# zzhuolun/conditioned-nerf-gan

Measured on AMD Instinct MI355X. Metric: rays/sec at 128x128x64spp ShapeNetCar, higher is better.
Workload: dtype f32; 1 GPU; ImplicitGenerator3d.forward SHORTSIREN_FG hidden 256, 128x128 rays x 64 coarse + 64 fine samples, feature volume 32x64^3, batch 8/GPU, hierarchical, white_back, relu, nerf_noise 0.0; img_size=128, num_steps=64, images_per_gpu=8, parallelism=image-batch data parallel x1, no data-path collective

## Files before the change

### conditioned-nerf-gan_amd/_lib.py

```python
import ctypes as C
import os

HERE = os.path.dirname(os.path.abspath(__file__))
LIB_PATH = os.path.join(HERE, "libcnerf_hip.so")

MAX_LAYERS = 16
MAX_LEVELS = 4
ABI_VERSION = 10
F_HIERARCHICAL, F_WHITE_BACK, F_LAST_BACK, F_SOFTPLUS, F_SIGMOID_RGB, F_INPUT_XYZ = 1, 2, 4, 8, 16, 32
F_NO_VOLUME = 128
PREC_FP32, PREC_FP16, PREC_FP16X3 = 0, 1, 2
PREC_CODE = {"fp32": PREC_FP32, "fp16": PREC_FP16, "fp16x3": PREC_FP16X3}
LAYER_FILM, LAYER_SINE, LAYER_RES, LAYER_PFILM = 0, 1, 2, 3
LAYER_CODE = {"film": LAYER_FILM, "sine": LAYER_SINE, "res": LAYER_RES, "pfilm": LAYER_PFILM}


class Cfg(C.Structure):
    _fields_ = [("B", C.c_int32), ("R", C.c_int32), ("S", C.c_int32), ("V", C.c_int32), ("C", C.c_int32),
                ("H", C.c_int32), ("L", C.c_int32), ("layer_kind", C.c_int32 * MAX_LAYERS),
                ("ray_start", C.c_float), ("ray_end", C.c_float), ("voxel_length", C.c_float),
                ("noise_std", C.c_float), ("flags", C.c_uint32), ("fov_deg", C.c_double),
                ("n_levels", C.c_int32), ("level_V", C.c_int32 * MAX_LEVELS), ("level_C", C.c_int32 * MAX_LEVELS),
                ("precision", C.c_int32), ("philox", C.c_uint32), ("philox_offset", C.c_uint32), ("philox_seed", C.c_uint64),
                ("drop_p", C.c_float), ("reserved0", C.c_uint32)]
# ... 33 lines not shown

class Rng(C.Structure):
    _fields_ = [("u_strat", C.c_void_p), ("eps_coarse", C.c_void_p), ("u_fine", C.c_void_p), ("eps_final", C.c_void_p),
                ("fine_z", C.c_void_p), ("drop_coarse", C.c_void_p), ("drop_fine", C.c_void_p)]


AUX_FIELDS = ("coarse_points", "coarse_z", "coarse_rgb_sigma", "coarse_weights", "cdf", "inds", "fine_z",
              "fine_rgb_sigma", "sort_idx", "final_weights", "fine_points")


class Act16(C.Structure):
    _fields_ = [("feat", C.c_void_p), ("h", C.c_void_p), ("c", C.c_void_p), ("amax", C.c_void_p)]


class Aux(C.Structure):
    _fields_ = [(k, C.c_void_p) for k in AUX_FIELDS] + [("field_events", C.c_void_p * 4), ("act16", Act16 * 2)]


PROTOTYPES = {
    "cnerf_abi_version": (C.c_int, []),
    "cnerf_last_error": (C.c_char_p, []),
    "cnerf_philox_fill": (C.c_int, [C.c_uint64, C.c_uint32, C.c_uint32, C.c_int64, C.c_int32, C.c_void_p, C.c_void_p]),
    "cnerf_workspace_bytes": (C.c_int, [C.POINTER(Cfg), C.POINTER(C.c_size_t), C.POINTER(C.c_size_t), C.POINTER(C.c_size_t)]),
    "cnerf_fvol_channel_last": (C.c_int, [C.c_int32, C.c_int32, C.c_int32, C.c_void_p, C.c_void_p, C.c_void_p]),
    "cnerf_fvol_channel_first": (C.c_int, [C.c_int32, C.c_int32, C.c_int32, C.c_void_p, C.c_void_p, C.c_void_p]),
    "cnerf_pack_field": (C.c_int, [C.POINTER(Cfg), C.POINTER(FieldParams), C.c_void_p, C.c_void_p]),
    "cnerf_gather_features": (C.c_int, [C.POINTER(Cfg), C.c_void_p, C.c_void_p, C.c_int64, C.c_void_p, C.c_void_p]),
    "cnerf_weight_grad": (C.c_int, [C.c_int32, C.c_int64, C.c_int32, C.c_int32, C.c_void_p, C.c_void_p, C.c_void_p, C.c_void_p,
                                    C.c_void_p]),
    "cnerf_scatter_features": (C.c_int, [C.POINTER(Cfg), C.c_void_p, C.c_int64, C.c_void_p, C.c_void_p, C.c_void_p]),
    "cnerf_field_forward": (C.c_int, [C.POINTER(Cfg), C.POINTER(Volumes), C.c_void_p, C.c_void_p, C.c_void_p, C.c_void_p,
                                      C.c_int64, C.c_void_p, C.c_void_p]),
    "cnerf_composite": (C.c_int, [C.POINTER(Cfg), C.c_int64, C.c_int32, C.c_void_p, C.c_void_p, C.c_void_p, C.c_void_p,
                                  C.c_void_p, C.c_void_p, C.c_void_p]),
    "cnerf_resample": (C.c_int, [C.c_int64, C.c_int32, C.c_void_p, C.c_void_p, C.c_void_p, C.c_void_p, C.c_void_p,
                                 C.c_void_p, C.c_void_p]),
    "cnerf_render_forward": (C.c_int, [C.POINTER(Cfg), C.POINTER(Volumes), C.c_void_p, C.c_void_p, C.c_void_p, C.c_void_p,
                                       C.POINTER(Rng), C.c_void_p, C.c_void_p, C.POINTER(Aux), C.c_void_p, C.c_void_p]),
    "cnerf_backward_bytes": (C.c_int, [C.POINTER(Cfg), C.POINTER(C.c_size_t)]),
    "cnerf_pack_field_transposed": (C.c_int, [C.POINTER(Cfg), C.POINTER(FieldParams), C.c_void_p, C.c_void_p]),
    "cnerf_merge_composite_backward": (C.c_int, [C.POINTER(Cfg)] + [C.c_void_p] * 10),
    "cnerf_field_backward": (C.c_int, [C.POINTER(Cfg), C.c_int32, C.c_int32, C.c_int32, C.POINTER(Volumes)] + [C.c_void_p] * 14 +
                             [C.POINTER(Volumes), C.c_void_p, C.c_void_p]),
    "cnerf_weight_grad16": (C.c_int, [C.c_int32, C.c_int64, C.c_int32, C.c_int32, C.c_int32] + [C.c_void_p] * 6),
    "cnerf_backward16_bytes": (C.c_int, [C.POINTER(Cfg), C.POINTER(C.c_size_t)]),
    "cnerf_pack_field_chain16": (C.c_int, [C.POINTER(Cfg), C.POINTER(FieldParams), C.c_void_p, C.c_void_p]),
# ... 83 lines not shown
```

### conditioned-nerf-gan_amd/csrc/cnerf_abi.hip

```cpp
#include <math.h>
#include <stdarg.h>
#include <stdio.h>
#include <stdlib.h>
#include <string.h>

#include "cnerf_kernels.hpp"

using namespace cnerf;

namespace {

thread_local char g_err[256] = "";

int fail(int code, const char* fmt, ...) {
    va_list ap;
    va_start(ap, fmt);
    vsnprintf(g_err, sizeof(g_err), fmt, ap);
    va_end(ap);
    return code;
}

int hip_fail(hipError_t e, const char* what) {
    return fail(CNERF_ELAUNCH, "%s: %s", what, hipGetErrorString(e));
}
// ... 264 lines not shown
    int H, film_stride;
    const float* film(const float* t, int m, int b0) const { return film_of[m] >= 0 ? t + (size_t)b0 * film_stride + (size_t)film_of[m] * H : nullptr; }
    float* film(float* t, int m, int b0) const { return film_of[m] >= 0 ? t + (size_t)b0 * film_stride + (size_t)film_of[m] * H : nullptr; }
};
int matrix_set(const cnerf_cfg* cfg, const cnerf_field_params* P, const cnerf_field_param_grads* G, const char* who, MatrixSet& ms) {
    int nm = 0, nfilm = 0;
    for (int l = 0; l < cfg->L; ++l) {
        const bool res = cfg->layer_kind[l] == CNERF_LAYER_RES;
        if (!P->w[l] || !P->b[l] || (res && (!P->w2[l] || !P->b2[l]))) return fail(CNERF_EINVAL, "%s: parameters of layer %d are NULL", who, l);
        ms.W[nm] = P->w[l]; ms.b[nm] = P->b[l]; ms.dW[nm] = G ? G->w[l] : nullptr; ms.db[nm] = G ? G->b[l] : nullptr;
        ms.film_of[nm] = cfg->layer_kind[l] == CNERF_LAYER_FILM ? nfilm++ : -1;
        ++nm;
        if (res) {
            ms.W[nm] = P->w2[l]; ms.b[nm] = P->b2[l]; ms.dW[nm] = G ? G->w2[l] : nullptr; ms.db[nm] = G ? G->b2[l] : nullptr;
            ms.film_of[nm] = -1;
            ++nm;
        }
    }
    ms.H = cfg->H;
    ms.film_stride = counts_of(cfg).n_film * cfg->H;
    return CNERF_OK;
}

struct ForwardLayout {
    size_t c_rs, f_rs, c_z, f_z;
    size_t fold, packed_img;
    long long layer_floats;
    size_t img16, fold16, rowf;
    size_t total;
};
ForwardLayout forward_layout(const cnerf_cfg* c) {
    const PackedLayout pl = packed_layout(c);
    const NetCounts nc = counts_of(c);
    const size_t N = (size_t)c->B * c->R * c->R * c->S, B = c->B, H = c->H, NT = H / 32, mats = nc.n_mats;
    ForwardLayout F{};
    size_t off = 0;
    auto take = [&](size_t bytes) { const size_t o = off; off += align256(bytes); return o; };
    F.c_rs = take(N * 4 * sizeof(float));
    F.f_rs = take(N * 4 * sizeof(float));
    F.c_z = take(N * sizeof(float));
    F.f_z = take(N * sizeof(float));
    if (c->precision != CNERF_PREC_FP32 && c->layer_kind[0] != CNERF_LAYER_PFILM) {
        F.img16 = take(B * pl.weight_floats * sizeof(float));
        F.fold16 = take(B * mats * (H + 1) * sizeof(float));
        F.rowf = take(B * mats * H * sizeof(float));
    } else {
        F.layer_floats = (long long)((NT * nc.n_in + (mats - 1) * NT * NT) * 1024);
        F.fold = take(4 * B * mats * H * sizeof(float));
        F.packed_img = take(B * (size_t)F.layer_floats * sizeof(float));
    }
    F.total = off;
    return F;
}

FieldArgs storing_args(const FieldArgs& a, long long n_points, void* feat, void* h, void* c, float* amax, void* scratch) {
    FieldArgs s = a;
    s.rgb_sigma = (float*)scratch;
    s.act_points = n_points;
    s.act_feat = (float*)feat;
    s.act_h = (float*)h;
    s.act_c = (float*)c;
    s.act_amax = amax;
    s.act_tb16 = 1;
    return s;
}

int field_backward_run(FieldArgs fa, const cnerf_cfg* cfg, long long n_points, const float* packed_t, const float* grad_out, const float* saved_out,
                       float* act_feat, float* act_h, float* act_c, float* act_g, float* act_go, hipStream_t stream) {
    fa.rgb_sigma = act_go;
    fa.act_points = n_points;
    fa.act_feat = act_feat;
    fa.act_h = act_h;
    fa.act_c = act_c;
    if (hipError_t e = launch_forward(fa, cfg, stream)) return hip_fail(e, "field kernel (activation store)");
    fa.packed_t = packed_t;
    fa.grad_out = grad_out;
    fa.saved_out = saved_out;
    fa.act_g = act_g;
    fa.act_go = act_go;
    if (hipError_t e = launch_field_backward(fa, cfg->H, stream)) return hip_fail(e, "field backward kernel");
    return CNERF_OK;
}

}

extern "C" {

int cnerf_abi_version(void) { return CNERF_ABI_VERSION; }

const char* cnerf_last_error(void) { return g_err; }

int cnerf_philox_fill(uint64_t seed, uint32_t offset, uint32_t stream_id, int64_t n, int32_t normal, float* out, void* stream) {
    g_err[0] = 0;
    if (!out || n < 1 || stream_id > 3) return fail(CNERF_EINVAL, "philox_fill: bad argument (stream_id 0..3)");
    const PhiloxKey k{1u, offset, (uint32_t)(seed & 0xffffffffull), (uint32_t)(seed >> 32)};
    if (hipError_t e = launch_philox_fill(k, stream_id, (long long)n, normal, out, (hipStream_t)stream)) return hip_fail(e, "philox_fill");
    return CNERF_OK;
}

int cnerf_workspace_bytes(const cnerf_cfg* cfg, size_t* packed, size_t* fvol_cl, size_t* fwd_ws) {
    g_err[0] = 0;
    if (int rc = check_cfg(cfg, fwd_ws != nullptr)) return rc;
    if (packed) *packed = align256(packed_layout(cfg).total * sizeof(float));
    if (fvol_cl) {
        size_t fl = 0;
        for (int i = 0; i < n_levels_of(cfg); ++i) fl += (size_t)cfg->B * level_floats(cfg, i);
        *fvol_cl = align256(fl * sizeof(float));
    }
    if (fwd_ws) *fwd_ws = forward_layout(cfg).total;
    return CNERF_OK;
}

int cnerf_fvol_channel_last(int32_t B, int32_t C, int32_t V, const float* fvol_cf, float* fvol_cl, void* stream) {
// ... 185 lines not shown
    const ForwardLayout F = forward_layout(cfg);
    char* ws = (char*)workspace;
    float* c_rs = (float*)(ws + F.c_rs);
    float* f_rs = (float*)(ws + F.f_rs);
    float* c_z = (float*)(ws + F.c_z);
    float* f_z = (float*)(ws + F.f_z);
    if (aux) {
        if (aux->coarse_rgb_sigma) c_rs = aux->coarse_rgb_sigma;
        if (aux->fine_rgb_sigma) f_rs = aux->fine_rgb_sigma;
        if (aux->coarse_z) c_z = aux->coarse_z;
        if (aux->fine_z) f_z = aux->fine_z;
    }

    FieldArgs fa;
    if (int rc = fill_field_args(fa, cfg, vols, nullptr, packed, freq, phase)) return rc;
    set_points(fa, cfg->B, npi);
    fa.cam2world = cam2world;
    if (cfg->precision == CNERF_PREC_FP32 && cfg->layer_kind[0] != CNERF_LAYER_PFILM && cfg->drop_p == 0.0f) {
        float* fold = (float*)(ws + F.fold);
        float* packed_img = (float*)(ws + F.packed_img);
        if (hipError_t e = launch_fold_film(fa, cfg->B, cfg->H, fold, stream)) return hip_fail(e, "fold_film");
        fa.fold = fold;
        fa.fold_images = cfg->B;
        if (hipError_t e = launch_scale_packed(fa, cfg->B, cfg->H, fold, F.layer_floats, packed_img, stream)) return hip_fail(e, "scale_packed");
        fa.packed_img = packed_img;
        fa.packed_img_stride = F.layer_floats;
    }
    if (cfg->precision != CNERF_PREC_FP32 && cfg->layer_kind[0] != CNERF_LAYER_PFILM) {
        void* img = ws + F.img16;
        float* fold16 = (float*)(ws + F.fold16);
        float* rowf = (float*)(ws + F.rowf);
        const long long img_elems = (long long)packed_layout(cfg).weight_floats * 2;
        if (hipError_t e = (cfg->precision == CNERF_PREC_FP16 ? launch_fold_h1 : launch_fold_h3)(fa, cfg->B, cfg->H, img, fold16, rowf, img_elems, stream))
            return hip_fail(e, "fold16");
        fa.packed_img = (const float*)img;
        fa.packed_img_stride = img_elems / 8;
        fa.fold = fold16;
        fa.fold_images = cfg->B;
    }
    fa.mode = FIELD_MODE_COARSE;
    fa.u_strat = rng->u_strat;
    fa.rgb_sigma = c_rs;
    fa.z_out = c_z;
    fa.points_out = aux ? aux->coarse_points : nullptr;
    auto mark = [&](int i) {
        if (aux && aux->field_events[i]) (void)hipEventRecord((hipEvent_t)aux->field_events[i], stream);
    };
    const bool keep = aux && aux->act16[0].h;
    if (keep) {
// ... 1376 lines not shown
```

### conditioned-nerf-gan_amd/csrc/cnerf_kernels.hpp

```cpp
#pragma once
#include <hip/hip_runtime.h>
#include <stdint.h>

#include <type_traits>

#include "../../include/cnerf.h"
#include "cnerf_dev.hpp"

namespace cnerf {

enum { FIELD_MODE_POINTS = 0, FIELD_MODE_COARSE = 1, FIELD_MODE_FINE = 2 };

struct FieldArgs {
    int n_in;
    int in_level[8];
    int in_chan[8];
    const float* lvl_vol[CNERF_MAX_LEVELS];
    float* lvl_grad[CNERF_MAX_LEVELS];
    int lvl_V[CNERF_MAX_LEVELS];
    int lvl_C[CNERF_MAX_LEVELS];
    const float* packed;
    const float* bias;
    const float* freq;
    const float* phase;
    const float* points;
    const float* cam2world;
    const float* u_strat;
    const float* fine_z;
    float* rgb_sigma;
    float* z_out;
    float* points_out;
    void* unused;
    long long act_points;
    float* act_feat;
    float* act_h;
    float* act_c;
    int act_tb16;
    float* act_amax;
    const float* packed_t;
    const float* grad_out;
    const float* saved_out;
    float* act_g;
    float* act_go;
    float* gin;
    long long n_per_image;
    long long tiles_per_image;
    long long total_tiles;
    RayGeom geom;
    float half_voxel;
    int L;
    int n_mats;
    int film_stride;
    int bias_floats;
    uint32_t flags;
    int mode;
// ... 29 lines not shown
    return (blocks + 7) / 8 * 8;
}

template <typename Args>
inline hipError_t launch_per_cu(void (*kernel)(Args), const FieldArgs& f, size_t lds_bytes, size_t lds_attr_bytes, const Args& args, hipStream_t stream) {
    if (hipError_t e = hipFuncSetAttribute((const void*)kernel, hipFuncAttributeMaxDynamicSharedMemorySize, (int)lds_attr_bytes)) return e;
    hipLaunchKernelGGL(kernel, dim3(one_block_per_cu_grid(f)), dim3(256), lds_bytes, stream, args);
    return hipGetLastError();
}

template <typename F>
inline hipError_t dispatch_nt(int H, F f) {
    switch (H / 32) {
        case 2: return f(std::integral_constant<int, 2>{});
        case 4: return f(std::integral_constant<int, 4>{});
        case 8: return f(std::integral_constant<int, 8>{});
        default: return hipErrorInvalidValue;
    }
}

hipError_t launch_fill(float* dst, float value, int n, hipStream_t stream);
hipError_t launch_pack_matrix(const float* w, int n_out, int K_real, int OT, float* dst, hipStream_t stream);
hipError_t launch_fold_film(const FieldArgs& a, int B, int H, float* out, hipStream_t stream);
hipError_t launch_scale_packed(const FieldArgs& a, int B, int H, const float* mh, long long layer_floats, float* out, hipStream_t stream);
hipError_t launch_field(const FieldArgs& a, int H, hipStream_t stream);
hipError_t launch_field_h3(const FieldArgs& a, int H, hipStream_t stream);
hipError_t launch_field_h1(const FieldArgs& a, int H, hipStream_t stream);
hipError_t launch_fold_h3(const FieldArgs& a, int B, int H, void* img, float* fold, float* rowf, long long img_elems, hipStream_t stream);
hipError_t launch_fold_h1(const FieldArgs& a, int B, int H, void* img, float* fold, float* rowf, long long img_elems, hipStream_t stream);
hipError_t launch_pack_h1(const float* w, int n_out, int K_real, int OT, bool k_outer, void* dst, float* inv_scale_slot, float* wmax_slot,
                          hipStream_t stream, long long t_stride = 0);
hipError_t launch_pack_h3(const float* w, int n_out, int K_real, int OT, bool k_outer, void* dst, float* inv_scale_slot, float* wmax_slot,
                          hipStream_t stream, long long t_stride = 0);
hipError_t launch_field_pw3(const FieldArgs& a, int H, hipStream_t stream);
hipError_t launch_field_pw1(const FieldArgs& a, int H, hipStream_t stream);
hipError_t launch_pw16_consts(const cnerf_field_params* p, int L, int H, const float* inv_s, float* consts, hipStream_t stream);
hipError_t launch_field_backward(const FieldArgs& a, int H, hipStream_t stream);
hipError_t launch_pack_head_t(const float* w, int H, float* dst, hipStream_t stream);
hipError_t launch_pack_head(const float* w, int H, float* dst, hipStream_t stream);
hipError_t launch_pack_matrix_t(const float* w, int n_rows_w, int n_cols_w, int OT, float* dst, hipStream_t stream);

struct CompositeArgs {
    const float* rgb_sigma;
    const float* z;
    const float* eps;
    float* rgb;
    float* dist;
// ... 276 lines not shown
```

### conditioned-nerf-gan_amd/csrc/field_kernel.hip

```cpp
#include "cnerf_dev.hpp"
#include "cnerf_kernels.hpp"
#include "field_common.hpp"

namespace cnerf {


__global__ void pack_matrix_kernel(const float* __restrict__ w, int n_out, int K_real, int K, int OT, float* __restrict__ dst) {
    const int KT = K / 32;
    const int total = OT * KT * 4 * 64 * 4;
    for (int idx = blockIdx.x * blockDim.x + threadIdx.x; idx < total; idx += gridDim.x * blockDim.x) {
        const int e = idx & 3;
        const int lane = (idx >> 2) & 63;
        const int g = (idx >> 8) & 3;
        const int rest = idx >> 10;
        const int tk = rest % KT, t = rest / KT;
        const int row = 32 * t + (lane & 31);
        const int col = 32 * tk + 8 * g + 4 * (lane >> 5) + e;
        dst[idx] = (row < n_out && col < K_real) ? w[(size_t)row * K_real + col] : 0.0f;
    }
}

__global__ void pack_head_kernel(const float* __restrict__ w, int H, float* __restrict__ dst) {
    const int total = (H / 2) * 64;
    const int idx = blockIdx.x * blockDim.x + threadIdx.x;
// ... 2 lines not shown
        const int sreg = 4 * q + e, t = sreg >> 4, r = sreg & 15, h = lane >> 5;
        const int ch = 32 * t + 8 * (r >> 2) + 4 * h + (r & 3);
        dst[idx] = w[(size_t)(lane & 3) * H + ch];
    }
}

template <int NT>
struct Act {
    f32x16 v[NT];
};

constexpr int RING = 6;


enum { EPI_FILM = 0, EPI_FILM_RES = 1 };

__device__ __forceinline__ float folded_sine(float pre, float mh, float ml, float k) {
    const float n = __builtin_rintf(pre * mh);
    return __builtin_amdgcn_sinf(__builtin_fmaf(pre, mh, -n) + k);
}

template <int WFOLD>
__device__ __forceinline__ float wfolded_sine(float u) {
    return __builtin_amdgcn_sinf(WFOLD == 1 ? __builtin_amdgcn_fractf(u) : u - __builtin_rintf(u));
}

template <int EPI, bool STORE>
__device__ __forceinline__ float epilogue_one(float acc, float res, float fr, float ph, float& cs) {
    float pre = acc;
    if (EPI == EPI_FILM_RES) pre = res + pre;
    if (STORE) {
        float sn;
        sincos_pi_reduced(fr * pre + ph, sn, cs);
        return sn;
    }
    return sin_pi_reduced(fr * pre + ph);
}

__device__ __forceinline__ void store_tile_rows(float* __restrict__ row , int t, int h, const f32x16& v) {
#pragma unroll
    for (int g = 0; g < 4; ++g) {
        f32x4 q;
#pragma unroll
        for (int e = 0; e < 4; ++e) q[e] = v[4 * g + e];
        *reinterpret_cast<f32x4*>(row + 32 * t + 8 * g + 4 * h) = q;
    }
}
// ... 155 lines not shown
    asm volatile("" : "+v"(wl));
#pragma unroll
    for (int t = 0; t < NT; ++t) {
#pragma unroll
        for (int g = 0; g < 4; ++g) {
#pragma unroll
            for (int e = 0; e < 4; ++e) {
                const f32x4 w = wl[(size_t)(t * 4) * 64 + 8 * g + e];
                y[t][4 * g + e] = __builtin_fmaf(w[2], pz, __builtin_fmaf(w[1], py, __builtin_fmaf(w[0], px, y[t][4 * g + e])));
            }
            __builtin_amdgcn_sched_barrier(0);
        }
    }
}


template <int NT, bool HAS_RES, bool STORE, bool DROP, bool FOLD = false, int WFOLD = 0, bool NOVOL = false>
__global__ __launch_bounds__(256) void field_tile_kernel(FieldArgs a) {
    const int lane = threadIdx.x & 63;
    const int j = lane & 31, h = lane >> 5;
    constexpr int H = NT * 32;
    constexpr size_t TILE4 = 4 * 64;
    constexpr bool BUF = WFOLD != 0 && !HAS_RES;

    __shared__ f32x4 s_head[NT * 4 * 64];
    {
        const f32x4* head_w = reinterpret_cast<const f32x4*>(a.packed) + ((size_t)NT * a.n_in + (size_t)(a.n_mats - 1) * NT * NT) * TILE4;
        for (int i = threadIdx.x; i < NT * 4 * 64; i += 256) s_head[i] = head_w[i];
        __syncthreads();
    }

    TileRange tr = tile_range(a.total_tiles);
    if constexpr (BUF) {
        const unsigned long long bv = (unsigned long long)tr.begin;
        tr.begin = (long long)(((unsigned long long)__builtin_amdgcn_readfirstlane((unsigned)(bv >> 32)) << 32) | __builtin_amdgcn_readfirstlane((unsigned)bv));
    }
    auto point_of = [&](long long tile, int& b_, long long& nn_, bool& valid_) {
        b_ = (int)(tile / a.tiles_per_image);
        const long long n = (tile - (long long)b_ * a.tiles_per_image) * 32 + j;
        valid_ = n < a.n_per_image;
        nn_ = valid_ ? n : (a.n_per_image - 1);
    };
    int b = 0;
    long long nn = 0;
    bool valid = false;
    float px = 0.f, py = 0.f, pz = 0.f;
// ... 35 lines not shown
            for (int g = 1; g < 4; ++g) *reinterpret_cast<f32x4*>(fo + 8 * g) = f32x4{0.f, 0.f, 0.f, 0.f};
        }
#pragma unroll
        for (int t = 0; t < NT; ++t) y.v[t] = ChanStream<BUF>(bias, H, h).tile(t);
        if constexpr (NOVOL) {
            layer0_xyz<NT>(wp, px, py, pz, y.v, h);
        } else
        for (int tk = 0; tk < a.n_in; ++tk) {
            const f32x16 feat = (AHEAD && tk == 0) ? lookup_tile_reduce(a, 0, ahead, px, py, pz) : input_tile(a, b, tk, px, py, pz, h);
            if (STORE) {
                float* fo = a.act_feat + gpt * (32 * a.n_in) + 32 * tk + 4 * h;
#pragma unroll
                for (int g = 0; g < 4; ++g) {
                    f32x4 q;
#pragma unroll
                    for (int e = 0; e < 4; ++e) q[e] = feat[4 * g + e];
                    *reinterpret_cast<f32x4*>(fo + 8 * g) = q;
                }
            }
            layer0_accumulate<NT, BUF>(wp, a.n_in, tk, feat, y.v, lane);
        }
        {
            const bool film = a.layer_kind[0] == CNERF_LAYER_FILM;
            film_all<NT, STORE, DROP, FOLD, WFOLD, BUF>(y.v, x.v, (FOLD || film) ? freq : ones, (FOLD || film) ? phase : zeros, h, row_h, row_c, &a, drop_gp, fml);
            if (STORE) {
                row_h += act_layer;
                row_c += act_layer;
            }
            wp += (size_t)NT * a.n_in * TILE4;
            bias += H;
            if (FOLD || film) {
                freq += H;
                phase += H;
                if (FOLD) fml += H;
            }
        }
        asm volatile("" :: "v"(x.v[0][0]), "v"(x.v[NT - 1][15]));
        for (int l = 1; l < a.L; ++l) {
            const int kind = a.layer_kind[l];
            if (!HAS_RES || kind != CNERF_LAYER_RES) {
                const bool film = kind == CNERF_LAYER_FILM;
                ++drop_d;
                mlp_matrix<NT, NT, EPI_FILM, STORE, DROP, FOLD, WFOLD, BUF>(wp, bias, (FOLD || film) ? freq : ones, (FOLD || film) ? phase : zeros, x.v,
                                                                       nullptr, y.v, lane, h, row_h, row_c, &a, drop_gp, drop_d, fml);
                if (STORE) {
                    row_h += act_layer;
                    row_c += act_layer;
                }
                wp += (size_t)NT * NT * TILE4;
                bias += H;
                if (FOLD || film) {
                    freq += H;
                    phase += H;
                    if (FOLD) fml += H;
                }
#pragma unroll
                for (int t = 0; t < NT; ++t) x.v[t] = y.v[t];
                asm volatile("" :: "v"(x.v[0][0]), "v"(x.v[NT - 1][15]));
            } else {
                mlp_matrix<NT, NT, EPI_FILM, STORE, false, FOLD, WFOLD, BUF>(wp, bias, FOLD ? freq : ones, FOLD ? phase : zeros, x.v, nullptr, y.v, lane, h,
                                                                        row_h, row_c, nullptr, 0, 0, fml);
                if (STORE) {
                    row_h += act_layer;
                    row_c += act_layer;
                }
                wp += (size_t)NT * NT * TILE4;
                bias += H;
                if (FOLD) {
                    freq += H;
                    phase += H;
                    fml += H;
                }
                mlp_matrix<NT, NT, EPI_FILM_RES, STORE, false, FOLD, WFOLD, BUF>(wp, bias, FOLD ? freq : ones, FOLD ? phase : zeros, y.v, x.v, x.v, lane, h,
                                                                            row_h, row_c, nullptr, 0, 0, fml);
                if (FOLD) {
                    freq += H;
                    phase += H;
                    fml += H;
                }
                if (STORE) {
                    row_h += act_layer;
                    row_c += act_layer;
                }
                wp += (size_t)NT * NT * TILE4;
                bias += H;
            }
        }

        float nx, ny, nz;
        tile_point_finish(a, nb, nnn, raw_next, nvalid, h, has_next, nx, ny, nz);
        if constexpr (AHEAD) lookup_tile_issue(a, nb, 0, nx, ny, nz, h, ahead);

        {
            const float* head_bias = WFOLD ? a.bias + (size_t)a.n_mats * H : bias;
            const f32x4 acc = head_forward<NT>(s_head, head_bias, x.v, lane);
            if (valid && h == 0) {
// ... 456 lines not shown
}

struct FoldMap {
    int film_of[2 * CNERF_MAX_LAYERS];
};
__global__ void fold_film_kernel(const float* __restrict__ freq, const float* __restrict__ phase, const float* __restrict__ bias, FoldMap map,
                                 int B, int n_mats, int H, int film_stride, float* __restrict__ out) {
    const long long n = (long long)B * n_mats * H;
    const long long i = (long long)blockIdx.x * blockDim.x + threadIdx.x;
    if (i < n) {
        const int ch = (int)(i % H), m = (int)((i / H) % n_mats), b = (int)(i / ((long long)H * n_mats));
        const int f = map.film_of[m];
        const double fr = f >= 0 ? (double)freq[(size_t)b * film_stride + (size_t)f * H + ch] : 1.0;
        const double ph = f >= 0 ? (double)phase[(size_t)b * film_stride + (size_t)f * H + ch] : 0.0;
        const double M = fr * 0.15915494309189533577;
        const float mh = (float)M;
        out[i] = mh;
        out[n + i] = (float)(M - (double)mh);
        out[2 * n + i] = (float)(ph * 0.15915494309189533577);
        out[3 * n + i] = (float)(M * (double)bias[(size_t)m * H + ch] + ph * 0.15915494309189533577);
    }
}

__global__ void scale_packed_kernel(const float* __restrict__ packed, const float* __restrict__ mh, const float* __restrict__ ml, int n_in, int NT,
                                    int n_mats, long long layer_floats, float* __restrict__ out) {
    const int b = blockIdx.y;
    const int H = NT * 32;
    const long long l0 = (long long)NT * n_in * 1024, lh = (long long)NT * NT * 1024;
    for (long long idx = (long long)blockIdx.x * blockDim.x + threadIdx.x; idx < layer_floats; idx += (long long)gridDim.x * blockDim.x) {
        int m;
        long long li;
        int KT;
        if (idx < l0) {
            m = 0;
            li = idx;
            KT = n_in;
        } else {
            m = 1 + (int)((idx - l0) / lh);
            li = (idx - l0) - (long long)(m - 1) * lh;
            KT = NT;
        }
        const int lane = (int)((li >> 2) & 63);
        const long long rest = li >> 10;
        const int t = (int)(rest / KT);
        const int row = 32 * t + (lane & 31);
        const size_t mi = ((size_t)b * n_mats + m) * H + row;
        out[(size_t)b * layer_floats + idx] = (float)((double)packed[idx] * ((double)mh[mi] + (double)ml[mi]));
    }
}

hipError_t launch_scale_packed(const FieldArgs& a, int B, int H, const float* mh, long long layer_floats, float* out, hipStream_t stream) {
    long long bx = (layer_floats + 255) / 256;
    if (bx > 1024) bx = 1024;
    const float* ml = mh + (size_t)B * a.n_mats * H;
    hipLaunchKernelGGL(scale_packed_kernel, dim3((unsigned)bx, (unsigned)B), dim3(256), 0, stream, a.packed, mh, ml, a.n_in, H / 32, a.n_mats, layer_floats,
                       out);
    return hipGetLastError();
}

hipError_t launch_fold_film(const FieldArgs& a, int B, int H, float* out, hipStream_t stream) {
    FoldMap map;
    int m = 0, films = 0;
    for (int l = 0; l < a.L; ++l) {
        if (a.layer_kind[l] == CNERF_LAYER_RES) {
            map.film_of[m++] = -1;
            map.film_of[m++] = -1;
        } else {
            map.film_of[m++] = a.layer_kind[l] == CNERF_LAYER_FILM ? films++ : -1;
        }
    }
    const long long n = (long long)B * a.n_mats * H;
    hipLaunchKernelGGL(fold_film_kernel, dim3((unsigned)((n + 255) / 256)), dim3(256), 0, stream, a.freq, a.phase, a.bias, map, B, a.n_mats, H,
                       a.film_stride, out);
    return hipGetLastError();
}

hipError_t launch_pack_matrix(const float* w, int n_out, int K_real, int OT, float* dst, hipStream_t stream) {
    const int K = (K_real + 31) / 32 * 32;
    const int total = OT * (K / 32) * 4 * 64 * 4;
// ... 52 lines not shown
        case 2: return launch_field_backward_res<2>(a, stream);
        case 4: return launch_field_backward_res<4>(a, stream);
        case 8: return launch_field_backward_res<8>(a, stream);
        default: return hipErrorInvalidValue;
    }
}

template <int NT, bool HAS_RES, bool STORE, bool DROP, bool FOLD = false, int WFOLD = 0, bool NOVOL = false>
static hipError_t launch_field_tile(const FieldArgs& a, hipStream_t stream) {
    if (NOVOL) {
        if (a.n_in != 1 || a.in_level[0] >= 0) return hipErrorInvalidValue;
    } else if (a.n_in < 1 || a.in_level[0] < 0) return hipErrorInvalidValue;
    const int blocks = field_grid((const void*)field_tile_kernel<NT, HAS_RES, STORE, DROP, FOLD, WFOLD, NOVOL>, a.total_tiles);
    hipLaunchKernelGGL((field_tile_kernel<NT, HAS_RES, STORE, DROP, FOLD, WFOLD, NOVOL>), dim3(blocks), dim3(256), 0, stream, a);
    return hipGetLastError();
}

template <int NT, bool HAS_RES, bool NOVOL = false>
static hipError_t launch_field_nt(const FieldArgs& a, hipStream_t stream) {
    if (a.drop_scale != 0.0f)
        return a.act_h ? launch_field_tile<NT, HAS_RES, true, true, false, 0, NOVOL>(a, stream) : launch_field_tile<NT, HAS_RES, false, true, false, 0, NOVOL>(a, stream);
    if (a.fold && a.packed_img && !a.act_h) {
        if constexpr (HAS_RES) return launch_field_tile<NT, true, false, false, true, 2, NOVOL>(a, stream);
        else return a.freq ? launch_field_tile<NT, false, false, false, true, 1, NOVOL>(a, stream) : launch_field_tile<NT, false, false, false, true, 2, NOVOL>(a, stream);
    }
    if constexpr (!NOVOL)
        if (a.fold && !a.act_h) return launch_field_tile<NT, HAS_RES, false, false, true>(a, stream);
    return a.act_h ? launch_field_tile<NT, HAS_RES, true, false, false, 0, NOVOL>(a, stream) : launch_field_tile<NT, HAS_RES, false, false, false, 0, NOVOL>(a, stream);
}

template <int NT>
static hipError_t launch_field_res(const FieldArgs& a, hipStream_t stream) {
    if (no_volume(a)) return has_res(a) ? launch_field_nt<NT, true, true>(a, stream) : launch_field_nt<NT, false, true>(a, stream);
    return has_res(a) ? launch_field_nt<NT, true>(a, stream) : launch_field_nt<NT, false>(a, stream);
}

template <int NT, bool STORE, bool DROP>
static hipError_t launch_field_pw(const FieldArgs& a, hipStream_t stream) {
    const int blocks = field_grid((const void*)field_pw_kernel<NT, STORE, DROP>, a.total_tiles);
    hipLaunchKernelGGL((field_pw_kernel<NT, STORE, DROP>), dim3(blocks), dim3(256), 0, stream, a);
    return hipGetLastError();
}

template <int NT>
static hipError_t launch_field_pw_nt(const FieldArgs& a, hipStream_t stream) {
    if (a.drop_scale != 0.0f) return a.act_h ? launch_field_pw<NT, true, true>(a, stream) : launch_field_pw<NT, false, true>(a, stream);
    return a.act_h ? launch_field_pw<NT, true, false>(a, stream) : launch_field_pw<NT, false, false>(a, stream);
// ... 21 lines not shown
```

### conditioned-nerf-gan_amd/ops.py

```python
import ctypes as C
import weakref
from types import SimpleNamespace
from typing import NamedTuple, Optional

import torch
import torch.nn.functional as F

from . import _lib as L

_pack_cache = weakref.WeakKeyDictionary()


def clear_pack_cache():
    _pack_cache.clear()


def _stream():
    return C.c_void_p(torch.cuda.current_stream().cuda_stream)


def _f32(t):
    if t is None:
        return None
    if t.dtype != torch.float32:
# ... 228 lines not shown
    for i, bufs in enumerate(act16):
        aux.act16[i].feat, aux.act16[i].h, aux.act16[i].c = (t.data_ptr() for t in bufs[:3])
        if len(bufs) > 3:
            aux.act16[i].amax = bufs[3].data_ptr()
    return aux


AUX_SHAPES = {
    "coarse_points": lambda B, P, S, n: ((B, P, S, 3), torch.float32),
    "coarse_z": lambda B, P, S, n: ((B, P, S), torch.float32),
    "coarse_rgb_sigma": lambda B, P, S, n: ((B, P, S, 4), torch.float32),
    "coarse_weights": lambda B, P, S, n: ((B, P, S), torch.float32),
    "cdf": lambda B, P, S, n: ((B, P, S - 1), torch.float32),
    "inds": lambda B, P, S, n: ((B, P, S), torch.int32),
    "fine_z": lambda B, P, S, n: ((B, P, S), torch.float32),
    "fine_rgb_sigma": lambda B, P, S, n: ((B, P, S, 4), torch.float32),
    "sort_idx": lambda B, P, S, n: ((B, P, 2 * S), torch.int32),
    "final_weights": lambda B, P, S, n: ((B, P, n), torch.float32),
    "fine_points": lambda B, P, S, n: ((B, P, S, 3), torch.float32),
}
HIER_ONLY = {"coarse_weights", "cdf", "inds", "fine_z", "fine_rgb_sigma", "sort_idx", "fine_points"}


def render_forward(net, fvol, freq, phase, cam2world, img_size, fov, ray_start, ray_end, num_steps, hierarchical,
                   clamp_mode, noise_std, white_back=False, last_back=False, rng: Optional[dict] = None,
                   want_aux=False, fvol_is_channel_last=False, field_events=None, aux_keys=None, act16=None):
    cam2world = _f32(cam2world)
    B, R, S = cam2world.shape[0], int(img_size), int(num_steps)
    P = R * R
    n = 2 * S if hierarchical else S
    dev = cam2world.device
    levels = [_f32(v) for v in as_levels(fvol)] if fvol_is_channel_last else channel_last_levels(fvol)
    cfg = make_cfg(net, B, levels, R, S, fov, ray_start, ray_end, noise_std, hierarchical, white_back,
                   last_back, clamp_mode, philox=(rng or {}).get("philox"), drop=drop_of(rng))
    vs = volumes_struct(levels)
    packed = pack_field(net, cfg)
    _, _, ws_bytes = sizes(cfg)
    ws = torch.empty(ws_bytes, dtype=torch.uint8, device=dev)
    pixels = torch.empty((B, 3, R, R), dtype=torch.float32, device=dev)
    depth = torch.empty((B, R, R), dtype=torch.float32, device=dev)
    r, keep = _rng_struct(rng or {}, ("u_strat", "eps_coarse", "u_fine", "eps_final", "fine_z", "drop_coarse", "drop_fine"))
    aux_t, aux_s = {}, None
    if want_aux or aux_keys:
        aux_s = L.Aux()
        for k in (L.AUX_FIELDS if want_aux else aux_keys):
            if not hierarchical and k in HIER_ONLY:
                continue
            shape, dt = AUX_SHAPES[k](B, P, S, n)
            aux_t[k] = torch.empty(shape, dtype=dt, device=dev)
            setattr(aux_s, k, aux_t[k].data_ptr())
    if field_events is not None:
        aux_s = aux_s if aux_s is not None else L.Aux()
        for i, ev in enumerate(field_events):
            aux_s.field_events[i] = ev
    if act16 is not None:
        aux_s = _act16_aux(act16, aux_s)
    L.check(L.lib().cnerf_render_forward(C.byref(cfg), C.byref(vs), L.ptr(packed), L.ptr(_f32(freq)), L.ptr(_f32(phase)),
                                         L.ptr(cam2world), C.byref(r), L.ptr(pixels), L.ptr(depth),
                                         C.byref(aux_s) if aux_s is not None else None, L.ptr(ws), _stream()),
            "cnerf_render_forward")
    return pixels, depth, aux_t


SAVED_KEYS = ("coarse_rgb_sigma", "coarse_z", "fine_rgb_sigma", "fine_z")


def pack_field_transposed(net, cfg):
    return _cached_pack(net, cfg, "transposed", lambda: _abi_bytes("cnerf_backward_bytes", cfg), "cnerf_pack_field_transposed", torch.float32)


PHASE_TIMER = None
ACT_BUDGET_BYTES = 128 << 30


def backward_precision_of(net):
    p = getattr(net, "backward_precision", "fp32")
    if p not in ("fp32", "fp16"):
        raise L.CnerfError(f"unknown backward precision {p!r}")
    return p


def n_matrices(net):
    return sum(2 if k == "res" else 1 for k in net.spec.layers)
# ... 508 lines not shown
```

### include/cnerf.h

```cpp
#ifndef CNERF_H
#define CNERF_H

#include <stddef.h>
#include <stdint.h>

#ifdef __cplusplus
extern "C" {
#endif

#define CNERF_ABI_VERSION 10

#define CNERF_OK 0
#define CNERF_EINVAL (-22)
#define CNERF_ENOSYS (-38)
#define CNERF_ELAUNCH (-5)

#define CNERF_MAX_LAYERS 16
#define CNERF_MAX_LEVELS 4

#define CNERF_F_HIERARCHICAL (1u << 0)
#define CNERF_F_WHITE_BACK (1u << 1)
#define CNERF_F_LAST_BACK (1u << 2)
#define CNERF_F_SOFTPLUS (1u << 3)
#define CNERF_F_SIGMOID_RGB (1u << 4)
// ... 72 lines not shown
    float* coarse_rgb_sigma;
    float* coarse_weights;
    float* cdf;
    int32_t* inds;
    float* fine_z;
    float* fine_rgb_sigma;
    int32_t* sort_idx;
    float* final_weights;
    float* fine_points;
    void* field_events[4];
    struct {
        void* feat;
        void* h;
        void* c;
        void* amax;
    } act16[2];
} cnerf_aux;

int cnerf_abi_version(void);
int cnerf_philox_fill(uint64_t seed, uint32_t offset, uint32_t stream_id, int64_t n, int32_t normal, float* out, void* stream);
const char* cnerf_last_error(void);

int cnerf_workspace_bytes(const cnerf_cfg* cfg, size_t* packed, size_t* fvol_cl, size_t* fwd_ws);

int cnerf_fvol_channel_last(int32_t B, int32_t C, int32_t V, const float* fvol_cf, float* fvol_cl, void* stream);
int cnerf_fvol_channel_first(int32_t B, int32_t C, int32_t V, const float* fvol_cl, float* fvol_cf, void* stream);

int cnerf_pack_field(const cnerf_cfg* cfg, const cnerf_field_params* params, float* packed, void* stream);

int cnerf_gather_features(const cnerf_cfg* cfg, const float* fvol_cl, const float* points, int64_t n_per_image,
                          float* feat, void* stream);

int cnerf_field_forward(const cnerf_cfg* cfg, const cnerf_volumes* vols, const float* packed, const float* freq,
                        const float* phase, const float* points, int64_t n_per_image, float* rgb_sigma, void* stream);

int cnerf_composite(const cnerf_cfg* cfg, int64_t rays, int32_t n, const float* rgb_sigma, const float* z,
                    const float* eps, float* rgb, float* dist, float* weights, void* stream);

int cnerf_resample(int64_t rays, int32_t S, const float* z, const float* weights, const float* u, float* fine_z,
                   int32_t* inds, float* cdf, void* stream);

int cnerf_render_forward(const cnerf_cfg* cfg, const cnerf_volumes* vols, const float* packed, const float* freq,
                         const float* phase, const float* cam2world, const cnerf_rng* rng, float* pixels,
                         float* depth, const cnerf_aux* aux, void* workspace, void* stream);


// ... 148 lines not shown
```

Before: 2.563 million rays/s.

## Skip sine range reduction when folded-weight bound proves arguments are small

The scale_packed kernel now computes, per image, an L1-norm upper bound on the hidden-layer sine arguments (sum of |W| plus |bias| per row) and atomically maxes it into a workspace word. The field kernel is launched in both a bounded variant (WFOLD 3/4), which calls the hardware sine directly without fract/rint range reduction, and the original variant. Each variant checks the device-side bound and exits early if it is not the matching case. This removes per-activation range-reduction work in the hidden layers when the bound holds. The cost is an extra launch whose blocks exit immediately, extra reduction work in scale_packed, and reliance on the hardware sine's accuracy for arguments up to the bound.

```diff
diff --git a/conditioned-nerf-gan_amd/_lib.py b/conditioned-nerf-gan_amd/_lib.py
--- a/conditioned-nerf-gan_amd/_lib.py
+++ b/conditioned-nerf-gan_amd/_lib.py
@@ -79,6 +79,7 @@
     "cnerf_last_error": (C.c_char_p, []),
     "cnerf_philox_fill": (C.c_int, [C.c_uint64, C.c_uint32, C.c_uint32, C.c_int64, C.c_int32, C.c_void_p, C.c_void_p]),
     "cnerf_workspace_bytes": (C.c_int, [C.POINTER(Cfg), C.POINTER(C.c_size_t), C.POINTER(C.c_size_t), C.POINTER(C.c_size_t)]),
+    "cnerf_forward_sine_bound_offset": (C.c_int, [C.POINTER(Cfg), C.POINTER(C.c_size_t)]),
     "cnerf_fvol_channel_last": (C.c_int, [C.c_int32, C.c_int32, C.c_int32, C.c_void_p, C.c_void_p, C.c_void_p]),
     "cnerf_fvol_channel_first": (C.c_int, [C.c_int32, C.c_int32, C.c_int32, C.c_void_p, C.c_void_p, C.c_void_p]),
     "cnerf_pack_field": (C.c_int, [C.POINTER(Cfg), C.POINTER(FieldParams), C.c_void_p, C.c_void_p]),
diff --git a/conditioned-nerf-gan_amd/csrc/cnerf_abi.hip b/conditioned-nerf-gan_amd/csrc/cnerf_abi.hip
--- a/conditioned-nerf-gan_amd/csrc/cnerf_abi.hip
+++ b/conditioned-nerf-gan_amd/csrc/cnerf_abi.hip
@@ -310,9 +310,15 @@
     return CNERF_OK;
 }
 
+bool bounded_sine_enabled() {
+    const char* s = getenv("CNERF_F32_BOUNDED_SINE");
+    return !(s && !strcmp(s, "0"));
+}
+
 struct ForwardLayout {
     size_t c_rs, f_rs, c_z, f_z;
     size_t fold, packed_img;
+    size_t sine_bound;
     long long layer_floats;
     size_t img16, fold16, rowf;
     size_t total;
@@ -336,6 +342,7 @@
         F.layer_floats = (long long)((NT * nc.n_in + (mats - 1) * NT * NT) * 1024);
         F.fold = take(4 * B * mats * H * sizeof(float));
         F.packed_img = take(B * (size_t)F.layer_floats * sizeof(float));
+        F.sine_bound = take(sizeof(uint32_t));
     }
     F.total = off;
     return F;
@@ -377,6 +384,16 @@
 int cnerf_abi_version(void) { return CNERF_ABI_VERSION; }
 
 const char* cnerf_last_error(void) { return g_err; }
+
+int cnerf_forward_sine_bound_offset(const cnerf_cfg* cfg, size_t* offset) {
+    g_err[0] = 0;
+    if (int rc = check_cfg(cfg, true)) return rc;
+    if (!offset) return fail(CNERF_EINVAL, "forward_sine_bound_offset: NULL argument");
+    if (cfg->precision != CNERF_PREC_FP32 || cfg->layer_kind[0] == CNERF_LAYER_PFILM || cfg->drop_p != 0.0f)
+        return fail(CNERF_EINVAL, "forward_sine_bound_offset: only the fp32 forward on folded weights (no per-point FiLM, no dropout) bounds its sine arguments");
+    *offset = forward_layout(cfg).sine_bound;
+    return CNERF_OK;
+}
 
 int cnerf_philox_fill(uint64_t seed, uint32_t offset, uint32_t stream_id, int64_t n, int32_t normal, float* out, void* stream) {
     g_err[0] = 0;
@@ -608,9 +625,12 @@
         if (hipError_t e = launch_fold_film(fa, cfg->B, cfg->H, fold, stream)) return hip_fail(e, "fold_film");
         fa.fold = fold;
         fa.fold_images = cfg->B;
-        if (hipError_t e = launch_scale_packed(fa, cfg->B, cfg->H, fold, F.layer_floats, packed_img, stream)) return hip_fail(e, "scale_packed");
+        uint32_t* sine_bound = (uint32_t*)(ws + F.sine_bound);
+        if (hipError_t e = hipMemsetAsync(sine_bound, 0, sizeof(uint32_t), stream)) return hip_fail(e, "memset");
+        if (hipError_t e = launch_scale_packed(fa, cfg->B, cfg->H, fold, F.layer_floats, packed_img, sine_bound, stream)) return hip_fail(e, "scale_packed");
         fa.packed_img = packed_img;
         fa.packed_img_stride = F.layer_floats;
+        fa.sine_bound = bounded_sine_enabled() ? sine_bound : nullptr;
     }
     if (cfg->precision != CNERF_PREC_FP32 && cfg->layer_kind[0] != CNERF_LAYER_PFILM) {
         void* img = ws + F.img16;
diff --git a/conditioned-nerf-gan_amd/csrc/cnerf_kernels.hpp b/conditioned-nerf-gan_amd/csrc/cnerf_kernels.hpp
--- a/conditioned-nerf-gan_amd/csrc/cnerf_kernels.hpp
+++ b/conditioned-nerf-gan_amd/csrc/cnerf_kernels.hpp
@@ -30,7 +30,7 @@
     float* rgb_sigma;
     float* z_out;
     float* points_out;
-    void* unused;
+    const uint32_t* sine_bound;
     long long act_points;
     float* act_feat;
     float* act_h;
@@ -106,7 +106,8 @@
 hipError_t launch_fill(float* dst, float value, int n, hipStream_t stream);
 hipError_t launch_pack_matrix(const float* w, int n_out, int K_real, int OT, float* dst, hipStream_t stream);
 hipError_t launch_fold_film(const FieldArgs& a, int B, int H, float* out, hipStream_t stream);
-hipError_t launch_scale_packed(const FieldArgs& a, int B, int H, const float* mh, long long layer_floats, float* out, hipStream_t stream);
+hipError_t launch_scale_packed(const FieldArgs& a, int B, int H, const float* mh, long long layer_floats, float* out, uint32_t* sine_bound,
+                               hipStream_t stream);
 hipError_t launch_field(const FieldArgs& a, int H, hipStream_t stream);
 hipError_t launch_field_h3(const FieldArgs& a, int H, hipStream_t stream);
 hipError_t launch_field_h1(const FieldArgs& a, int H, hipStream_t stream);
diff --git a/conditioned-nerf-gan_amd/csrc/field_kernel.hip b/conditioned-nerf-gan_amd/csrc/field_kernel.hip
--- a/conditioned-nerf-gan_amd/csrc/field_kernel.hip
+++ b/conditioned-nerf-gan_amd/csrc/field_kernel.hip
@@ -48,7 +48,12 @@
 
 template <int WFOLD>
 __device__ __forceinline__ float wfolded_sine(float u) {
+    if (WFOLD == 3) return __builtin_amdgcn_sinf(u);
     return __builtin_amdgcn_sinf(WFOLD == 1 ? __builtin_amdgcn_fractf(u) : u - __builtin_rintf(u));
+}
+
+__device__ __forceinline__ bool sine_bounded(uint32_t bits) {
+    return __builtin_bit_cast(float, bits) * (1.0f + 0x1p-12f) + 1.0f <= 250.0f;
 }
 
 template <int EPI, bool STORE>
@@ -250,6 +255,11 @@
     constexpr int H = NT * 32;
     constexpr size_t TILE4 = 4 * 64;
     constexpr bool BUF = WFOLD != 0 && !HAS_RES;
+    constexpr int W0 = WFOLD > 2 ? WFOLD - 2 : WFOLD, WH = WFOLD > 2 ? 3 : WFOLD;
+    if constexpr (BUF) {
+        const bool bounded = a.sine_bound && sine_bounded(*a.sine_bound);
+        if (bounded != (WFOLD > 2)) return;
+    }
 
     __shared__ f32x4 s_head[NT * 4 * 64];
     {
@@ -331,7 +341,7 @@
         }
         {
             const bool film = a.layer_kind[0] == CNERF_LAYER_FILM;
-            film_all<NT, STORE, DROP, FOLD, WFOLD, BUF>(y.v, x.v, (FOLD || film) ? freq : ones, (FOLD || film) ? phase : zeros, h, row_h, row_c, &a, drop_gp, fml);
+            film_all<NT, STORE, DROP, FOLD, W0, BUF>(y.v, x.v, (FOLD || film) ? freq : ones, (FOLD || film) ? phase : zeros, h, row_h, row_c, &a, drop_gp, fml);
             if (STORE) {
                 row_h += act_layer;
                 row_c += act_layer;
@@ -350,7 +360,7 @@
             if (!HAS_RES || kind != CNERF_LAYER_RES) {
                 const bool film = kind == CNERF_LAYER_FILM;
                 ++drop_d;
-                mlp_matrix<NT, NT, EPI_FILM, STORE, DROP, FOLD, WFOLD, BUF>(wp, bias, (FOLD || film) ? freq : ones, (FOLD || film) ? phase : zeros, x.v,
+                mlp_matrix<NT, NT, EPI_FILM, STORE, DROP, FOLD, WH, BUF>(wp, bias, (FOLD || film) ? freq : ones, (FOLD || film) ? phase : zeros, x.v,
                                                                        nullptr, y.v, lane, h, row_h, row_c, &a, drop_gp, drop_d, fml);
                 if (STORE) {
                     row_h += act_layer;
@@ -367,7 +377,7 @@
                 for (int t = 0; t < NT; ++t) x.v[t] = y.v[t];
                 asm volatile("" :: "v"(x.v[0][0]), "v"(x.v[NT - 1][15]));
             } else {
-                mlp_matrix<NT, NT, EPI_FILM, STORE, false, FOLD, WFOLD, BUF>(wp, bias, FOLD ? freq : ones, FOLD ? phase : zeros, x.v, nullptr, y.v, lane, h,
+                mlp_matrix<NT, NT, EPI_FILM, STORE, false, FOLD, WH, BUF>(wp, bias, FOLD ? freq : ones, FOLD ? phase : zeros, x.v, nullptr, y.v, lane, h,
                                                                         row_h, row_c, nullptr, 0, 0, fml);
                 if (STORE) {
                     row_h += act_layer;
@@ -380,7 +390,7 @@
                     phase += H;
                     fml += H;
                 }
-                mlp_matrix<NT, NT, EPI_FILM_RES, STORE, false, FOLD, WFOLD, BUF>(wp, bias, FOLD ? freq : ones, FOLD ? phase : zeros, y.v, x.v, x.v, lane, h,
+                mlp_matrix<NT, NT, EPI_FILM_RES, STORE, false, FOLD, WH, BUF>(wp, bias, FOLD ? freq : ones, FOLD ? phase : zeros, y.v, x.v, x.v, lane, h,
                                                                             row_h, row_c, nullptr, 0, 0, fml);
                 if (FOLD) {
                     freq += H;
@@ -883,39 +893,77 @@
     }
 }
 
-__global__ void scale_packed_kernel(const float* __restrict__ packed, const float* __restrict__ mh, const float* __restrict__ ml, int n_in, int NT,
-                                    int n_mats, long long layer_floats, float* __restrict__ out) {
+__device__ __forceinline__ uint32_t bound_bits(double u) {
+    u *= 1.0 + 0x1p-22;
+    float f = (float)u;
+    uint32_t bits = __builtin_bit_cast(uint32_t, f) & 0x7fffffffu;
+    if ((double)f < u) ++bits;
+    return bits;
+}
+
+__global__ __launch_bounds__(256) void scale_packed_kernel(const float* __restrict__ packed, const float* __restrict__ mh, const float* __restrict__ ml,
+                                                           const float* __restrict__ kb, int n_in, int NT, int n_mats, long long layer_floats,
+                                                           float* __restrict__ out, uint32_t* __restrict__ sine_bound) {
     const int b = blockIdx.y;
     const int H = NT * 32;
     const long long l0 = (long long)NT * n_in * 1024, lh = (long long)NT * NT * 1024;
-    for (long long idx = (long long)blockIdx.x * blockDim.x + threadIdx.x; idx < layer_floats; idx += (long long)gridDim.x * blockDim.x) {
-        int m;
-        long long li;
-        int KT;
-        if (idx < l0) {
-            m = 0;
-            li = idx;
-            KT = n_in;
-        } else {
-            m = 1 + (int)((idx - l0) / lh);
-            li = (idx - l0) - (long long)(m - 1) * lh;
-            KT = NT;
-        }
-        const int lane = (int)((li >> 2) & 63);
-        const long long rest = li >> 10;
-        const int t = (int)(rest / KT);
-        const int row = 32 * t + (lane & 31);
-        const size_t mi = ((size_t)b * n_mats + m) * H + row;
+    const int units = (n_mats - 1) * NT;
+    __shared__ double s_row[64];
+    if ((int)blockIdx.x < units) {
+        const int m = 1 + (int)blockIdx.x / NT, t = (int)blockIdx.x % NT;
+        const int lane = threadIdx.x >> 2;
+        const size_t mrow = ((size_t)b * n_mats + m) * H + 32 * t;
+        const double M = (double)mh[mrow + (lane & 31)] + (double)ml[mrow + (lane & 31)];
+        const long long base = l0 + (long long)(m - 1) * lh + (long long)t * NT * 1024 + threadIdx.x;
+        float* __restrict__ o = out + (size_t)b * layer_floats;
+        double sum = 0.0;
+#pragma unroll 8
+        for (int i = 0; i < NT * 4; ++i) {
+            const float w = (float)((double)packed[base + 256 * i] * M);
+            o[base + 256 * i] = w;
+            sum += (double)__builtin_fabsf(w);
+        }
+        sum += __shfl_xor(sum, 1);
+        sum += __shfl_xor(sum, 2);
+        if ((threadIdx.x & 3) == 0) s_row[lane] = sum;
+        __syncthreads();
+        if (threadIdx.x < 64) {
+            uint32_t bits = 0;
+            if (threadIdx.x < 32) {
+                const int r = threadIdx.x;
+                bits = bound_bits(s_row[r] + s_row[r + 32] + (double)__builtin_fabsf(kb[mrow + r]));
+                if (m == 1) {
+                    const uint32_t k0 = __builtin_bit_cast(uint32_t, kb[(size_t)b * n_mats * H + 32 * t + r]) & 0x7fffffffu;
+                    if (k0 >= 0x7f800000u) bits = k0;
+                }
+            }
+#pragma unroll
+            for (int d = 16; d >= 1; d >>= 1) {
+                const uint32_t other = (uint32_t)__shfl_xor((int)bits, d);
+                bits = other > bits ? other : bits;
+            }
+            if (threadIdx.x == 0 && sine_bound) atomicMax(sine_bound, bits);
+        }
+        return;
+    }
+    const long long first = (long long)((int)blockIdx.x - units) * 256 + threadIdx.x, step = (long long)((int)gridDim.x - units) * 256;
+    for (long long idx = first; idx < l0; idx += step) {
+        const int lane = (int)((idx >> 2) & 63);
+        const int t = (int)((idx >> 10) / n_in);
+        const size_t mi = (size_t)b * n_mats * H + 32 * t + (lane & 31);
         out[(size_t)b * layer_floats + idx] = (float)((double)packed[idx] * ((double)mh[mi] + (double)ml[mi]));
     }
 }
 
-hipError_t launch_scale_packed(const FieldArgs& a, int B, int H, const float* mh, long long layer_floats, float* out, hipStream_t stream) {
-    long long bx = (layer_floats + 255) / 256;
+hipError_t launch_scale_packed(const FieldArgs& a, int B, int H, const float* mh, long long layer_floats, float* out, uint32_t* sine_bound,
+                               hipStream_t stream) {
+    const int NT = H / 32;
+    long long bx = ((long long)NT * a.n_in * 1024 + 255) / 256;
     if (bx > 1024) bx = 1024;
-    const float* ml = mh + (size_t)B * a.n_mats * H;
-    hipLaunchKernelGGL(scale_packed_kernel, dim3((unsigned)bx, (unsigned)B), dim3(256), 0, stream, a.packed, mh, ml, a.n_in, H / 32, a.n_mats, layer_floats,
-                       out);
+    bx += (a.n_mats - 1) * NT;
+    const size_t n = (size_t)B * a.n_mats * H;
+    hipLaunchKernelGGL(scale_packed_kernel, dim3((unsigned)bx, (unsigned)B), dim3(256), 0, stream, a.packed, mh, mh + n, mh + 3 * n, a.n_in, NT, a.n_mats,
+                       layer_floats, out, sine_bound);
     return hipGetLastError();
 }
 
@@ -1014,7 +1062,12 @@
         return a.act_h ? launch_field_tile<NT, HAS_RES, true, true, false, 0, NOVOL>(a, stream) : launch_field_tile<NT, HAS_RES, false, true, false, 0, NOVOL>(a, stream);
     if (a.fold && a.packed_img && !a.act_h) {
         if constexpr (HAS_RES) return launch_field_tile<NT, true, false, false, true, 2, NOVOL>(a, stream);
-        else return a.freq ? launch_field_tile<NT, false, false, false, true, 1, NOVOL>(a, stream) : launch_field_tile<NT, false, false, false, true, 2, NOVOL>(a, stream);
+        else {
+            if (a.sine_bound)
+                if (hipError_t e = a.freq ? launch_field_tile<NT, false, false, false, true, 3, NOVOL>(a, stream) : launch_field_tile<NT, false, false, false, true, 4, NOVOL>(a, stream))
+                    return e;
+            return a.freq ? launch_field_tile<NT, false, false, false, true, 1, NOVOL>(a, stream) : launch_field_tile<NT, false, false, false, true, 2, NOVOL>(a, stream);
+        }
     }
     if constexpr (!NOVOL)
         if (a.fold && !a.act_h) return launch_field_tile<NT, HAS_RES, false, false, true>(a, stream);
diff --git a/conditioned-nerf-gan_amd/ops.py b/conditioned-nerf-gan_amd/ops.py
--- a/conditioned-nerf-gan_amd/ops.py
+++ b/conditioned-nerf-gan_amd/ops.py
@@ -274,6 +274,16 @@
 HIER_ONLY = {"coarse_weights", "cdf", "inds", "fine_z", "fine_rgb_sigma", "sort_idx", "fine_points"}
 
 
+LAST_SINE_BOUND = None
+SINE_BOUND_LIMIT = 250.0
+
+
+def sine_bound_accepted(bound):
+    import numpy as np
+    b = np.float32(bound)
+    return bool(b * np.float32(1.0 + 2.0 ** -12) + np.float32(1.0) <= np.float32(SINE_BOUND_LIMIT))
+
+
 def render_forward(net, fvol, freq, phase, cam2world, img_size, fov, ray_start, ray_end, num_steps, hierarchical,
                    clamp_mode, noise_std, white_back=False, last_back=False, rng: Optional[dict] = None,
                    want_aux=False, fvol_is_channel_last=False, field_events=None, aux_keys=None, act16=None):
@@ -311,6 +321,11 @@
                                          L.ptr(cam2world), C.byref(r), L.ptr(pixels), L.ptr(depth),
                                          C.byref(aux_s) if aux_s is not None else None, L.ptr(ws), _stream()),
             "cnerf_render_forward")
+    if want_aux and cfg.precision == L.PREC_FP32 and net.spec.layers[0] != "pfilm" and not drop_of(rng):
+        global LAST_SINE_BOUND
+        off = C.c_size_t(0)
+        L.check(L.lib().cnerf_forward_sine_bound_offset(C.byref(cfg), C.byref(off)), "cnerf_forward_sine_bound_offset")
+        LAST_SINE_BOUND = ws[off.value:off.value + 4].view(torch.float32).clone()
     return pixels, depth, aux_t
 
 
diff --git a/include/cnerf.h b/include/cnerf.h
--- a/include/cnerf.h
+++ b/include/cnerf.h
@@ -118,6 +118,7 @@
 const char* cnerf_last_error(void);
 
 int cnerf_workspace_bytes(const cnerf_cfg* cfg, size_t* packed, size_t* fvol_cl, size_t* fwd_ws);
+int cnerf_forward_sine_bound_offset(const cnerf_cfg* cfg, size_t* offset);
 
 int cnerf_fvol_channel_last(int32_t B, int32_t C, int32_t V, const float* fvol_cf, float* fvol_cl, void* stream);
 int cnerf_fvol_channel_first(int32_t B, int32_t C, int32_t V, const float* fvol_cl, float* fvol_cf, void* stream);
```

Measured after the change: 2.576 million rays/s, median of 6. No clear change (+0.5%).
